# yellofi/SelectiveNet_for_semantic_segmentation_binary

Measured on AMD Instinct MI355X. Metric: train images/sec, SelectiveUNet_B 256x256 bs=128 (global), selective_loss s_lamb=2, higher is better.
Workload: dtype f32; 1 GPU; SelectiveUNet_B train step, global bs=128, 256x256, Adam lr=1e-3, s_lamb=2; model=SelectiveUNet_B, global_batch=128, per_gpu_batch=128, image=256, parallelism=dp1

## Files before the change

### selectivenet_for_semantic_segmentation_binary_amd/csrc/conv3x3.hip

```cpp
#include <cstdlib>

#include "gemm_common.h"

namespace selunet {

constexpr int TH = 16, TW = 16;
constexpr int HHT = TH + 2, HWT = TW + 2;
constexpr int HPIX = HHT * HWT;
constexpr int HTHREADS = 512;
constexpr int A_ROUNDS = (HPIX * 8 + HTHREADS - 1) / HTHREADS;
constexpr int AROWB = 160;
__device__ __forceinline__ int halo_off(int hp, int cc) { return hp * AROWB + ((cc ^ ((hp / HWT) & 1)) << 4); }

template <typename T, int BN, bool ONE_CHUNK>
__global__ void __launch_bounds__(HTHREADS, ONE_CHUNK ? 2 : 1)
conv3x3_halo_kernel(GatherArg g, const T* __restrict__ B, int N, int k_pad, EpiArg ep, int n_tiles, int tiles_x,
                    int tiles_y) {
  constexpr int E = 16 / sizeof(T);
  constexpr int CK = 128 / sizeof(T);
  constexpr int WAVES_N = BN / 64;
  constexpr int WAVES_M = 8 / WAVES_N;
  constexpr int WPIX = (TH * TW) / WAVES_M;
  constexpr int MT = WPIX / 32;
  constexpr int NT = 2;
// ... 1174 lines not shown
    __builtin_memcpy(&v, e, 16);
    return v;
  };
  uint4 rp[P_ROUNDS], rx[X_ROUNDS];
  auto load_tile = [&](int pt) __attribute__((always_inline)) {
    int img, y0, x0;
    tile_origin(pt, img, y0, x0);
#pragma unroll
    for (int r = 0; r < P_ROUNDS; ++r) {
      const int idx = r * 512 + tid;
      const int px = idx / (BI / 8), cc = idx % (BI / 8);
      const int y = min(y0 + px / WTW, H - 1), x = min(x0 + px % WTW, W - 1);
      rp[r] = *reinterpret_cast<const uint4*>(reinterpret_cast<const __bf16*>(pa.data) +
                                             (((int64_t)img * H + y) * W + x) * pa.C + i0 + cc * 8);
    }
#pragma unroll
    for (int r = 0; r < X_ROUNDS; ++r) {
      const int idx = r * 512 + tid;
      const int hp = min(idx >> 3, WHP - 1), cc = idx & 7;
      const int y = min(max(y0 - 1 + hp / WHW, 0), H - 1), x = min(max(x0 - 1 + hp % WHW, 0), W - 1);
      rx[r] = *reinterpret_cast<const uint4*>(reinterpret_cast<const __bf16*>(xa.data) +
                                             (((int64_t)img * H + y) * W + x) * xa.C + xc + cc * 8);
    }
  };
  auto store_tile = [&](int pt, int buf) __attribute__((always_inline)) {
    int img, y0, x0;
    tile_origin(pt, img, y0, x0);
#pragma unroll
    for (int r = 0; r < P_ROUNDS; ++r) {
      const int idx = r * 512 + tid;
      const int px = idx / (BI / 8), cc = idx % (BI / 8);
      uint4 v = make_uint4(0, 0, 0, 0);
      if (y0 + px / WTW < H && x0 + px % WTW < W)
        v = pa.scale ? apply(rp[r], Ks + cc * 8, Ks + BI + cc * 8, pa.relu) : rp[r];
      *reinterpret_cast<uint4*>(&Ps[buf][px][cc * 8]) = v;
    }
#pragma unroll
    for (int r = 0; r < X_ROUNDS; ++r) {
      const int idx = r * 512 + tid;
      if (idx < WHP * 8) {
        const int hp = idx >> 3, cc = idx & 7;
        const int y = y0 - 1 + hp / WHW, x = x0 - 1 + hp % WHW;
        uint4 v = make_uint4(0, 0, 0, 0);
        if ((unsigned)y < (unsigned)H && (unsigned)x < (unsigned)W)
          v = xa.scale ? apply(rx[r], Ks + 2 * BI + cc * 8, Ks + 2 * BI + 64 + cc * 8, xa.relu) : rx[r];
        *reinterpret_cast<uint4*>(&Xs[buf][hp][cc * 8]) = v;
      }
    }
  };

  f32x16 acc[NTAP];
#pragma unroll
  for (int t = 0; t < NTAP; ++t) acc[t] = f32x16{};

  load_tile((int)pt_begin);
  __syncthreads();
  store_tile((int)pt_begin, 0);
  __syncthreads();
  auto tile_loop = [&](auto ntc) __attribute__((always_inline)) {
    constexpr int NTP = decltype(ntc)::value;
    int buf = 0;
    for (int pt = (int)pt_begin; pt < (int)pt_end; ++pt) {
      const bool more = pt + 1 < (int)pt_end;
      load_tile(more ? pt + 1 : pt);
      __builtin_amdgcn_sched_barrier(0);
  #pragma unroll
      for (int ks = 0; ks < WTH; ++ks) {
        const int prow = ks * WTW + 8 * half + q4;
        const int pcol = wi * 32 + 16 * grp_hi + 4 * p4;
        s16x4 lo = __builtin_amdgcn_ds_read_tr16_b64_v4i16((__attribute__((address_space(3))) s16x4*)&Ps[buf][prow][pcol]);
        s16x4 hi = __builtin_amdgcn_ds_read_tr16_b64_v4i16((__attribute__((address_space(3))) s16x4*)&Ps[buf][prow + 4][pcol]);
        const bf16x8 af = __builtin_bit_cast(bf16x8, __builtin_shufflevector(lo, hi, 0, 1, 2, 3, 4, 5, 6, 7));
        const int xcol = wj * 32 + 16 * grp_hi + 4 * p4;
        constexpr int PF = 3;
        auto read_tap = [&](int t) __attribute__((always_inline)) {
          const int tap = min(tap0 + t, 8);
          const int dy = tap / 3, dx = tap - (tap / 3) * 3;
          const int xrow = (ks + dy) * WHW + 8 * half + dx + q4;
          s16x4 blo = __builtin_amdgcn_ds_read_tr16_b64_v4i16((__attribute__((address_space(3))) s16x4*)&Xs[buf][xrow][xcol]);
          s16x4 bhi = __builtin_amdgcn_ds_read_tr16_b64_v4i16((__attribute__((address_space(3))) s16x4*)&Xs[buf][xrow + 4][xcol]);
          return __builtin_bit_cast(bf16x8, __builtin_shufflevector(blo, bhi, 0, 1, 2, 3, 4, 5, 6, 7));
        };
        bf16x8 bfr[NTAP];
  #pragma unroll
        for (int t = 0; t < PF && t < NTAP; ++t) bfr[t] = read_tap(t);
        __builtin_amdgcn_sched_group_barrier(0x100, 2 + 2 * PF, 0);
  #pragma unroll
        for (int t = 0; t < NTAP; ++t) {
          if (t < NTP) acc[t] = __builtin_amdgcn_mfma_f32_32x32x16_bf16(af, bfr[t], acc[t], 0, 0, 0);
          __builtin_amdgcn_sched_group_barrier(0x008, 1, 0);
          if (t + PF < NTAP) {
            bfr[t + PF] = read_tap(t + PF);
            __builtin_amdgcn_sched_group_barrier(0x100, 2, 0);
          }
        }
      }
      if (more) store_tile(pt + 1, buf ^ 1);
      __syncthreads();
      buf ^= 1;
    }
  };
  if (TG == 1) tile_loop(std::integral_constant<int, 9>{});
  else if (tg == 0) tile_loop(std::integral_constant<int, 5>{});
  else tile_loop(std::integral_constant<int, 4>{});

  const int ctot = Q.Ctot;
#pragma unroll
  for (int t = 0; t < NTAP; ++t) {
    if (t < ntap) {
      const int tap = tap0 + t;
      const int j = tap * ctot + c0 + wj * 32 + l32;
#pragma unroll
      for (int r = 0; r < 16; ++r) {
        const int i = i0 + wi * 32 + (r & 3) + 8 * (r >> 2) + 4 * half;
        if (ws) ws[split * ws_stride + (int64_t)i * ldo + j] = acc[t][r];
        else atomicAdd(out + (int64_t)i * ldo + j, acc[t][r]);
      }
    }
  }
}

constexpr int XTH = 8, XTW = 8, XHW = XTW + 2, XHP = (XTH + 2) * XHW, XPIX = XTH * XTW;

template <int BI, int BNA = 0, bool TQ = false>
__global__ void __launch_bounds__(512, 1)
conv3x3_wgrad_x2_kernel(GatherArg P, GatherArg Q, int ldo, int co_tiles, int ci_chunks, int64_t tiles_per_split,
                        int tiles_x, int tiles_y, int64_t total_tiles, float* __restrict__ ws, int64_t ws_stride,
                        const float* __restrict__ amax_p, const float* __restrict__ amax_q0,
                        const float* __restrict__ amax_q1, WgradBnArg bn, unsigned* __restrict__ tq = nullptr) {
  constexpr int LDP = BI + 32;
  constexpr int LDX = 64 + 32;
  constexpr int TG = BI == 64 ? 2 : 1;
  constexpr int NTAP = TG == 1 ? 9 : 5;
  constexpr int P_ROUNDS = (XPIX * BI / 4) / 512;
  constexpr int X_ROUNDS = (XHP * 16 + 511) / 512;
  constexpr bool POOL = BNA == 2, HEADS = BNA == 3;
  constexpr int KX = BNA ? (HEADS ? 8 : 5) * BI : 2 * BI;
  constexpr int NWIN = XPIX * BI / 16;
  static_assert(P_ROUNDS * 512 == XPIX * BI / 4, "dY tile must split evenly over the threads");
  static_assert(!(POOL || HEADS) || (BI == 64 && NWIN <= 512), "pool / heads sources are BI = 64 forms");

  __shared__ __attribute__((aligned(16))) _Float16 Ps[2][2][XPIX][LDP];
  __shared__ __attribute__((aligned(16))) _Float16 Xs[2][2][XHP][LDX];
  __shared__ __attribute__((aligned(16))) float Ks[KX + 2 * 64];

  const int tid = threadIdx.x;
  const int lane = tid & 63, wave = tid >> 6;
  const int wj = wave & 1;
  const int wi = (wave >> 1) % (BI / 32);
  const int tg = (wave >> 1) / (BI / 32);
  const int tap0 = tg * 5;
  const int ntap = TG == 1 ? 9 : (tg == 0 ? 5 : 4);
  const int half = lane >> 5, l32 = lane & 31;
  const int grp_hi = (lane >> 4) & 1, q4 = (lane & 15) >> 2, p4 = lane & 3;

  const unsigned lb = xcd_remap(blockIdx.x, gridDim.x);
  const int cot = lb % co_tiles;
  const int rest = lb / co_tiles;
  const int cik = rest % ci_chunks;
  const int64_t split = rest / ci_chunks;
  const int i0 = cot * BI;
  const int c0 = cik * 64;
  const int ngroups = co_tiles * ci_chunks, grp = (int)(lb % (unsigned)ngroups);
  __shared__ int tq_slot[2];
  int pt_first, pt_second, pt_stop;
  if constexpr (TQ) {
    if (tid == 0) {
      const unsigned t = atomicAdd(tq + grp, 2u);
      tq_slot[0] = (int)min(t, (unsigned)total_tiles);
      tq_slot[1] = (int)min(t + 1u, (unsigned)total_tiles);
    }
    __syncthreads();
    pt_first = tq_slot[0];
    pt_second = tq_slot[1];
    pt_stop = (int)total_tiles;
  } else {
    pt_first = (int)(split * tiles_per_split);
    pt_second = pt_first + 1;
    pt_stop = (int)min(total_tiles, (int64_t)pt_first + tiles_per_split);
  }

  int xs_src = 0, xc = c0;
  if (Q.nsrc > 1 && xc >= Q.src[0].C) {
    xc -= Q.src[0].C;
    xs_src = 1;
  }
  const SrcArg xa = pick_src(Q, xs_src);
  const SrcArg& pa = P.src[0];
  const int H = P.h, W = P.w;
  float uns_p, uns_x;
  const float sp = x2_scale(amax_p[0], &uns_p);
  const float sx = x2_scale((xs_src ? amax_q1 : amax_q0)[0], &uns_x);

  if constexpr (BNA) {
    for (int k = tid; k < KX; k += 512) {
      const int c = i0 + (k % BI), C = P.Ctot;
      float v;
      switch (k / BI) {
        case 0: v = bn.scale[c]; break;
        case 1: v = bn.shift[c]; break;
        case 2: v = bn.coef[c]; break;
        case 3: v = bn.coef[2 * C + c] * bn.invstd[c]; break;
        case 4: v = bn.coef[C + c] - bn.coef[2 * C + c] * bn.invstd[c] * bn.mean[c]; break;
        default: {
          const int hd = k / BI - 5;
          v = hd < bn.nh ? bn.hw[hd * 64 + c] : 0.0f;
        }
      }
      Ks[k] = v;
    }
    if (tid < 128) {
      const int c = xc + (tid % 64);
      Ks[KX + tid] = xa.scale ? (tid < 64 ? xa.scale[c] : xa.shift[c]) : 0.0f;
    }
  } else if (tid < 2 * BI + 128) {
    float v;
    if (tid < 2 * BI) {
      const int c = i0 + (tid % BI);
      v = pa.scale ? (tid < BI ? pa.scale[c] : pa.shift[c]) : 0.0f;
    } else {
      const int c = xc + ((tid - 2 * BI) % 64);
      v = xa.scale ? (tid < 2 * BI + 64 ? xa.scale[c] : xa.shift[c]) : 0.0f;
    }
    Ks[tid] = v;
  }
  float dam = 0.0f;
  const bool dy_out = BNA && bn.dy != nullptr;

  constexpr int PPR = 512 / (BI / 4);
  const int hrem = H - (tiles_y - 1) * XTH, wrem = W - (tiles_x - 1) * XTW;
  const int pcc = tid % (BI / 4);
  unsigned tb = 0, p_off, g_off = 0, w_off = 0, x_off[X_ROUNDS];
  if constexpr (POOL) {
    const int wn = tid / (BI / 4), wyy = 2 * (wn / (XTW / 2)), wxx = 2 * (wn % (XTW / 2));
    p_off = (unsigned)((wyy * W + wxx) * pa.C + pcc * 4) * 4u;
    w_off = (unsigned)(((wyy / 2) * (W / 2) + wxx / 2) * pa.C + pcc * 4) * 4u;
    if (wyy >= hrem) tb |= 1u << 16;
    if (wxx >= wrem) tb |= 1u << 20;
#pragma unroll
    for (int k = 0; k < 4; ++k)
      if (((wyy + (k >> 1)) * XTW + wxx + (k & 1)) % ci_chunks == cik) tb |= 1u << (24 + k);
  } else {
    const int px = tid / (BI / 4), py = px / XTW, pxx = px % XTW;
    p_off = (unsigned)((py * W + pxx) * pa.C + pcc * 4) * 4u;
    if constexpr (HEADS) g_off = (unsigned)(py * W + pxx) * 4u;
    if (pxx >= wrem) tb |= 1u << 20;
#pragma unroll
    for (int r = 0; r < P_ROUNDS; ++r) {
      if (py + r * (PPR / XTW) >= hrem) tb |= 1u << (16 + r);
      if (BNA && (r * PPR + px) % ci_chunks == cik) tb |= 1u << (24 + r);
    }
  }
#pragma unroll
  for (int r = 0; r < X_ROUNDS; ++r) {
    const int hp = min((r * 512 + tid) >> 4, XHP - 1), hy = hp / XHW, hx = hp % XHW;
    x_off[r] = (unsigned)((hy * W + hx) * xa.C + (tid & 15) * 4) * 4u;
    tb |= (unsigned)((hy == 0) | (hy > hrem) << 1 | (hx == 0) << 2 | (hx > wrem) << 3) << (4 * r);
  }
  const unsigned p_rstride = (unsigned)((PPR / XTW) * W * pa.C) * 4u;
  const unsigned g_rstride = (unsigned)((PPR / XTW) * W) * 4u;
  const unsigned x_safe = (unsigned)((W + 1) * xa.C) * 4u;
  struct Geo {
    int64_t pix;
    int64_t hpix;
    unsigned em;
  };
  auto tile_geo = [&](int pt_) __attribute__((always_inline)) {
    const unsigned pt = (unsigned)__builtin_amdgcn_readfirstlane(pt_);
    const unsigned r2 = pt / (unsigned)tiles_x, tx = pt - r2 * (unsigned)tiles_x;
    const unsigned r3 = r2 / (unsigned)tiles_y, ty = r2 - r3 * (unsigned)tiles_y;
    Geo g;
    g.pix = ((int64_t)r3 * H + ty * XTH) * W + tx * XTW;
    g.hpix = POOL ? ((int64_t)r3 * (H / 2) + ty * (XTH / 2)) * (W / 2) + tx * (XTW / 2) : 0;
    g.em = (ty == 0 ? 0x1111u : 0u) | (ty == (unsigned)tiles_y - 1u ? 0x0f2222u : 0u) |
           (tx == 0 ? 0x4444u : 0u) | (tx == (unsigned)tiles_x - 1u ? 0x108888u : 0u);
    return g;
  };
  auto p_in = [&](const Geo& g, int r) __attribute__((always_inline)) {
    return (tb & g.em & ((POOL ? 1u << 16 : 1u << (16 + r)) | 1u << 20)) == 0;
  };
  auto x_in = [&](const Geo& g, int r) __attribute__((always_inline)) { return (tb & g.em & (0xfu << (4 * r))) == 0; };
  auto at = [&](const void* base, int64_t elems, unsigned off) __attribute__((always_inline)) {
    return reinterpret_cast<const char*>(reinterpret_cast<const float*>(base) + elems) + (size_t)off;
  };
  auto put = [&](float4 v, const float* sc, const float* sh, int relu, float s, _Float16* hp, _Float16* lp)
      __attribute__((always_inline)) {
    float f[4] = {v.x, v.y, v.z, v.w};
    f16x4 h, l;
#pragma unroll
    for (int j = 0; j < 4; ++j) {
      float t = f[j];
      if (sc) {
        t = t * sc[j] + sh[j];
        if (relu) t = fmaxf(t, 0.0f);
      }
      _Float16 a, b;
      x2_split(t * s, a, b);
      h[j] = a;
      l[j] = b;
    }
    *reinterpret_cast<f16x4*>(hp) = h;
    *reinterpret_cast<f16x4*>(lp) = l;
  };
  float4 rp[P_ROUNDS], rx[X_ROUNDS];
  float4 ry[BNA ? P_ROUNDS : 1];
  float rg[HEADS ? P_ROUNDS : 1][3];
  float4 wy[POOL ? 4 : 1], wk[POOL ? 4 : 1], wg;
  auto load_p = [&](const Geo& g, int r0, int r1) __attribute__((always_inline)) {
    const int64_t e0 = g.pix * pa.C + i0;
    if constexpr (POOL) {
      if (r0 == 0 && tid < NWIN) {
        const bool in = p_in(g, 0);
        const unsigned o = in ? p_off : 0u;
        const int64_t rs = (int64_t)W * pa.C;
        const int64_t ek[4] = {e0, e0 + pa.C, e0 + rs, e0 + rs + pa.C};
#pragma unroll
        for (int k = 0; k < 4; ++k) {
          wy[k] = *reinterpret_cast<const float4*>(at(bn.y, ek[k], o));
          wk[k] = bn.skip ? *reinterpret_cast<const float4*>(at(bn.skip, ek[k], o)) : make_float4(0, 0, 0, 0);
        }
        wg = *reinterpret_cast<const float4*>(at(bn.pooled, g.hpix * pa.C + i0, in ? w_off : 0u));
      }
      return;
    }
#pragma unroll
    for (int r = 0; r < P_ROUNDS; ++r) {
      if (r < r0 || r >= r1) continue;
      const bool in = p_in(g, r);
      const unsigned o = in ? p_off + r * p_rstride : 0u;
      if constexpr (HEADS) {
        const unsigned go = in ? g_off + r * g_rstride : 0u;
        rg[r][0] = *reinterpret_cast<const float*>(at(bn.g0, g.pix, go));
        rg[r][1] = bn.nh > 1 ? *reinterpret_cast<const float*>(at(bn.g1, g.pix, go)) : 0.0f;
        rg[r][2] = bn.nh > 1 ? *reinterpret_cast<const float*>(at(bn.g2, g.pix, go)) : 0.0f;
      } else {
        rp[r] = *reinterpret_cast<const float4*>(at(pa.data, e0, o));
      }
      if constexpr (BNA) ry[r] = *reinterpret_cast<const float4*>(at(bn.y, e0, o));
    }
  };
  auto load_x = [&](const Geo& g) __attribute__((always_inline)) {
    const int64_t e0 = (g.pix - W - 1) * xa.C + xc;
#pragma unroll
    for (int r = 0; r < X_ROUNDS; ++r)
      rx[r] = *reinterpret_cast<const float4*>(at(xa.data, e0, x_in(g, r) ? x_off[r] : x_safe));
  };
  auto store_p = [&](const Geo& tl, int buf, int r0, int r1) __attribute__((always_inline)) {
    const int64_t e0 = tl.pix * pa.C + i0;
    if constexpr (POOL) {
      if (r0 == 0 && tid < NWIN) {
        const int wi = tid / (BI / 4), cg = tid % (BI / 4);
        const int wyy = 2 * (wi / (XTW / 2)), wxx = 2 * (wi % (XTW / 2));
        const bool in = p_in(tl, 0);
        const f32x4 csc = *reinterpret_cast<const f32x4*>(Ks + cg * 4);
        const f32x4 csh = *reinterpret_cast<const f32x4*>(Ks + BI + cg * 4);
        const f32x4 ck0 = *reinterpret_cast<const f32x4*>(Ks + 2 * BI + cg * 4);
        const f32x4 ca = *reinterpret_cast<const f32x4*>(Ks + 3 * BI + cg * 4);
        const f32x4 cb = *reinterpret_cast<const f32x4*>(Ks + 4 * BI + cg * 4);
        const float yv[4][4] = {{wy[0].x, wy[0].y, wy[0].z, wy[0].w}, {wy[1].x, wy[1].y, wy[1].z, wy[1].w},
                                {wy[2].x, wy[2].y, wy[2].z, wy[2].w}, {wy[3].x, wy[3].y, wy[3].z, wy[3].w}};
        const float gv[4] = {wg.x, wg.y, wg.z, wg.w};
        int arg[4] = {0, 0, 0, 0};
#pragma unroll
        for (int e = 0; e < 4; ++e) {
          float best = fmaxf(yv[0][e] * csc[e] + csh[e], 0.0f);
#pragma unroll
          for (int k = 1; k < 4; ++k) {
            const float v = fmaxf(yv[k][e] * csc[e] + csh[e], 0.0f);
            if (v > best) {
              best = v;
              arg[e] = k;
            }
          }
        }
#pragma unroll
        for (int k = 0; k < 4; ++k) {
          float d[4] = {wk[k].x, wk[k].y, wk[k].z, wk[k].w};
          float o[4];
#pragma unroll
          for (int e = 0; e < 4; ++e) {
            if (arg[e] == k) d[e] += gv[e];
            o[e] = (yv[k][e] * csc[e] + csh[e] > 0.0f ? ck0[e] * d[e] : 0.0f) - cb[e] - ca[e] * yv[k][e];
          }
          const int py = wyy + (k >> 1), pxx = wxx + (k & 1), px = py * XTW + pxx;
          const float4 dv = in ? make_float4(o[0], o[1], o[2], o[3]) : make_float4(0, 0, 0, 0);
          if (dy_out && in && (tb & (1u << (24 + k)))) {
            const int64_t ek = e0 + ((k >> 1) * (int64_t)W + (k & 1)) * pa.C;
            *reinterpret_cast<float4*>(const_cast<char*>(at(bn.dy, ek, p_off))) = dv;
            dam = fmaxf(dam, fmaxf(fmaxf(fabsf(dv.x), fabsf(dv.y)), fmaxf(fabsf(dv.z), fabsf(dv.w))));
          }
          put(dv, nullptr, nullptr, 0, sp, &Ps[buf][0][px][cg * 4], &Ps[buf][1][px][cg * 4]);
        }
      }
      return;
    }
#pragma unroll
    for (int r = 0; r < P_ROUNDS; ++r) {
      if (r < r0 || r >= r1) continue;
      const int idx = r * 512 + tid;
      const int px = idx / (BI / 4), cc = idx % (BI / 4);
      const bool in = p_in(tl, r);
      if constexpr (BNA) {
        float g[4] = {rp[r].x, rp[r].y, rp[r].z, rp[r].w};
        const float yv[4] = {ry[r].x, ry[r].y, ry[r].z, ry[r].w};
        if constexpr (HEADS) {
          const f32x4 w0 = *reinterpret_cast<const f32x4*>(Ks + 5 * BI + cc * 4);
          const f32x4 w1 = *reinterpret_cast<const f32x4*>(Ks + 6 * BI + cc * 4);
          const f32x4 w2 = *reinterpret_cast<const f32x4*>(Ks + 7 * BI + cc * 4);
#pragma unroll
          for (int e = 0; e < 4; ++e) g[e] = w0[e] * rg[r][0] + w1[e] * rg[r][1] + w2[e] * rg[r][2];
        }
        const f32x4 csc = *reinterpret_cast<const f32x4*>(Ks + cc * 4);
        const f32x4 csh = *reinterpret_cast<const f32x4*>(Ks + BI + cc * 4);
        const f32x4 ck0 = *reinterpret_cast<const f32x4*>(Ks + 2 * BI + cc * 4);
        const f32x4 ca = *reinterpret_cast<const f32x4*>(Ks + 3 * BI + cc * 4);
        const f32x4 cb = *reinterpret_cast<const f32x4*>(Ks + 4 * BI + cc * 4);
        float o[4];
#pragma unroll
        for (int e = 0; e < 4; ++e)
          o[e] = (yv[e] * csc[e] + csh[e] > 0.0f ? ck0[e] * g[e] : 0.0f) - cb[e] - ca[e] * yv[e];
        const float4 d = in ? make_float4(o[0], o[1], o[2], o[3]) : make_float4(0, 0, 0, 0);
        if (dy_out && in && (tb & (1u << (24 + r)))) {
          *reinterpret_cast<float4*>(const_cast<char*>(at(bn.dy, e0 + r * (int64_t)(p_rstride / 4), p_off))) = d;
          dam = fmaxf(dam, fmaxf(fmaxf(fabsf(d.x), fabsf(d.y)), fmaxf(fabsf(d.z), fabsf(d.w))));
        }
        put(d, nullptr, nullptr, 0, sp, &Ps[buf][0][px][cc * 4], &Ps[buf][1][px][cc * 4]);
      } else {
        put(in ? rp[r] : make_float4(0, 0, 0, 0), pa.scale && in ? Ks + cc * 4 : nullptr, Ks + BI + cc * 4, pa.relu,
            sp, &Ps[buf][0][px][cc * 4], &Ps[buf][1][px][cc * 4]);
      }
    }
  };
  auto store_x = [&](const Geo& g, int buf) __attribute__((always_inline)) {
#pragma unroll
    for (int r = 0; r < X_ROUNDS; ++r) {
      const int idx = r * 512 + tid;
      if (idx < XHP * 16) {
        const int hp = idx >> 4, cc = idx & 15;
        const bool in = x_in(g, r);
        put(in ? rx[r] : make_float4(0, 0, 0, 0), xa.scale && in ? Ks + KX + cc * 4 : nullptr,
            Ks + KX + 64 + cc * 4, xa.relu, sx, &Xs[buf][0][hp][cc * 4], &Xs[buf][1][hp][cc * 4]);
      }
    }
  };

  f32x16 acc[NTAP];
#pragma unroll
  for (int t = 0; t < NTAP; ++t) acc[t] = f32x16{};

  if (pt_first < pt_stop) {
    const Geo g0 = tile_geo(pt_first);
    load_p(g0, 0, P_ROUNDS);
    load_x(g0);
    __syncthreads();
    store_p(g0, 0, 0, P_ROUNDS);
    store_x(g0, 0);
    __syncthreads();
  }
  typedef __attribute__((address_space(3))) s16x4 lds_s16x4;
  auto tr8 = [&](const _Float16* p0, const _Float16* p1) __attribute__((always_inline)) {
    s16x4 lo = __builtin_amdgcn_ds_read_tr16_b64_v4i16((lds_s16x4*)p0);
    s16x4 hi = __builtin_amdgcn_ds_read_tr16_b64_v4i16((lds_s16x4*)p1);
    return __builtin_bit_cast(f16x8, __builtin_shufflevector(lo, hi, 0, 1, 2, 3, 4, 5, 6, 7));
  };
  auto tile_loop = [&](auto ntc) __attribute__((always_inline)) {
    constexpr int NTP = decltype(ntc)::value;
    int buf = 0;
    int pt_tq = pt_second;
    for (int pt = pt_first; pt < pt_stop;) {
      const int ptn = TQ ? pt_tq : pt + 1;
      const bool more = ptn < pt_stop;
      unsigned claimed = 0;
      constexpr bool QSPLIT = BNA && BI == 128;
      constexpr int PH = QSPLIT ? P_ROUNDS / 2 : P_ROUNDS;
      const Geo gn = tile_geo(more ? ptn : pt);
      load_p(gn, 0, PH);
      __builtin_amdgcn_sched_barrier(0);
#pragma unroll
      for (int ks = 0; ks < XPIX / 16; ++ks) {
        if (QSPLIT && ks == 1) {
          if (more) store_p(gn, buf ^ 1, 0, PH);
          load_p(gn, PH, P_ROUNDS);
          __builtin_amdgcn_sched_barrier(0);
        }
        if (BI == 64 && ks == 1) {
          load_x(gn);
          __builtin_amdgcn_sched_barrier(0);
        }
        if (ks == (QSPLIT || BI == 64 ? 3 : 2)) {
          if (more) store_p(gn, buf ^ 1, QSPLIT ? PH : 0, P_ROUNDS);
          if (BI != 64) load_x(gn);
          __builtin_amdgcn_sched_barrier(0);
        }
        if constexpr (TQ) {
          if (ks == 0 && tid == 0) claimed = atomicAdd(tq + grp, 1u);
        }
        const int prow = ks * 16 + 8 * half + q4;
        const int pcol = wi * 32 + 16 * grp_hi + 4 * p4;
        const f16x8 ah = tr8(&Ps[buf][0][prow][pcol], &Ps[buf][0][prow + 4][pcol]);
        const f16x8 al = tr8(&Ps[buf][1][prow][pcol], &Ps[buf][1][prow + 4][pcol]);
        const int xcol = wj * 32 + 16 * grp_hi + 4 * p4;
        constexpr int PF = BI == 128 ? 1 : 2;
        struct Frag {
          f16x8 h, l;
        };
        auto read_tap = [&](int t) __attribute__((always_inline)) {
          constexpr int TAP0 = TG == 2 && NTP == 4 ? 5 : 0;
          const int tap = min(TAP0 + t, 8);
          const int dy = tap / 3, dx = tap - (tap / 3) * 3;
          const int xrow = (2 * ks + half + dy) * XHW + dx + q4;
          Frag f;
          f.h = tr8(&Xs[buf][0][xrow][xcol], &Xs[buf][0][xrow + 4][xcol]);
          f.l = tr8(&Xs[buf][1][xrow][xcol], &Xs[buf][1][xrow + 4][xcol]);
          return f;
        };
        Frag bfr[NTAP];
#pragma unroll
        for (int t = 0; t < PF && t < NTAP; ++t) bfr[t] = read_tap(t);
        __builtin_amdgcn_sched_group_barrier(0x100, 4 + 4 * PF, 0);
#pragma unroll
        for (int t = 0; t < NTAP; ++t) {
          if (t < NTP) {
            acc[t] = __builtin_amdgcn_mfma_f32_32x32x16_f16(ah, bfr[t].l, acc[t], 0, 0, 0);
            acc[t] = __builtin_amdgcn_mfma_f32_32x32x16_f16(al, bfr[t].h, acc[t], 0, 0, 0);
            acc[t] = __builtin_amdgcn_mfma_f32_32x32x16_f16(ah, bfr[t].h, acc[t], 0, 0, 0);
          }
          __builtin_amdgcn_sched_group_barrier(0x008, 3, 0);
          if (t + PF < NTAP) {
            bfr[t + PF] = read_tap(t + PF);
            __builtin_amdgcn_sched_group_barrier(0x100, 4, 0);
          }
        }
      }
      if constexpr (TQ) {
        if (tid == 0) tq_slot[buf] = (int)min(claimed, (unsigned)pt_stop);
      }
      if (more) store_x(gn, buf ^ 1);
      __syncthreads();
      if constexpr (TQ) pt_tq = tq_slot[buf];
      pt = ptn;
      buf ^= 1;
    }
  };
  if (TG == 1) tile_loop(std::integral_constant<int, 9>{});
  else if (tg == 0) tile_loop(std::integral_constant<int, 5>{});
  else tile_loop(std::integral_constant<int, 4>{});

  if constexpr (BNA) {
    if (bn.dy_amax) block_amax(bn.dy_amax, dam, Ks);
  }
  if constexpr (TQ) {
    const unsigned splits = gridDim.x / (unsigned)ngroups;
    if (tid == 0 && atomicAdd(tq + ngroups + grp, 1u) == splits - 1u) {
      atomicExch(tq + grp, 0u);
      atomicExch(tq + ngroups + grp, 0u);
    }
  }
  const float ofac = uns_p * uns_x;
  const int ctot = Q.Ctot;
#pragma unroll
  for (int t = 0; t < NTAP; ++t) {
    if (t < ntap) {
      const int tap = tap0 + t;
      const int j = tap * ctot + c0 + wj * 32 + l32;
#pragma unroll
      for (int r = 0; r < 16; ++r) {
        const int i = i0 + wi * 32 + (r & 3) + 8 * (r >> 2) + 4 * half;
        ws[split * ws_stride + (int64_t)i * ldo + j] = acc[t][r] * ofac;
      }
    }
  }
}

constexpr int FTH = 8, FTW = 8;

template <int BI, int WCO>
__global__ void __launch_bounds__(512, 1)
conv3x3_wgrad_halo_f32_kernel(GatherArg P, GatherArg Q, float* __restrict__ out, int ldo, int co_tiles,
                              int ci_chunks, int64_t tiles_per_split, int tiles_x, int tiles_y, int64_t total_tiles,
                              float* __restrict__ ws, int64_t ws_stride) {
  constexpr int CJ = 64;
  constexpr int WTH = FTH, WTW = FTW, WHW = FTW + 2, WPIXT = FTH * FTW, WHP = (FTH + 2) * (FTW + 2);
  constexpr int NT = 512;
  constexpr int MA = WCO / 32;
  constexpr int COH = BI / WCO;
  constexpr int TGN = 8 / (COH * 2);
  static_assert(TGN == 2 || TGN == 4, "8 waves = co groups x 2 ci halves x tap groups");
  constexpr int NTAP = TGN == 2 ? 5 : 3;
  constexpr int P_ROUNDS = (WPIXT * BI / 4) / NT;
  constexpr int X_ROUNDS = (WHP * (CJ / 4) + NT - 1) / NT;
  constexpr int KS = WPIXT / 2;
  constexpr int UNR = BI == 128 ? 2 : 4;
  static_assert(P_ROUNDS * NT == WPIXT * BI / 4, "dY tile must split evenly over the threads");

  __shared__ __attribute__((aligned(16))) float Ps[2][WPIXT][BI];
  __shared__ __attribute__((aligned(16))) float Xs[2][WHP][CJ];
  __shared__ float Ks[2 * BI + 2 * CJ];

  const int tid = threadIdx.x;
  const int lane = tid & 63, wave = tid >> 6;
  const int wj = wave & 1;
  const int wc = (wave >> 1) % COH;
  const int tg = (wave >> 1) / COH;
  const int tap0 = TGN == 2 ? tg * 5 : (tg == 0 ? 0 : 1 + 2 * tg);
  const int ntap = TGN == 2 ? (tg == 0 ? 5 : 4) : (tg == 0 ? 3 : 2);
  const int half = lane >> 5, l32 = lane & 31;

  const unsigned lb = xcd_remap(blockIdx.x, gridDim.x);
  const int cot = lb % co_tiles;
  const int rest = lb / co_tiles;
  const int cik = rest % ci_chunks;
  const int64_t split = rest / ci_chunks;
  const int i0 = cot * BI;
  const int c0 = cik * CJ;
  const int64_t pt_begin = split * tiles_per_split;
  const int64_t pt_end = min(total_tiles, pt_begin + tiles_per_split);
  if (pt_begin >= pt_end) return;

  int xs_src = 0, xc = c0;
  if (Q.nsrc > 1 && xc >= Q.src[0].C) {
    xc -= Q.src[0].C;
    xs_src = 1;
  }
  const SrcArg xa = pick_src(Q, xs_src);
  const SrcArg& pa = P.src[0];
  const int H = P.h, W = P.w;

  if (tid < 2 * BI + 2 * CJ) {
    float v;
    if (tid < 2 * BI) {
      const int c = i0 + (tid % BI);
      v = pa.scale ? (tid < BI ? pa.scale[c] : pa.shift[c]) : 0.0f;
    } else {
      const int c = xc + ((tid - 2 * BI) % CJ);
      v = xa.scale ? (tid < 2 * BI + CJ ? xa.scale[c] : xa.shift[c]) : 0.0f;
    }
    Ks[tid] = v;
  }

  auto tile_origin = [&](int pt, int& img, int& y0, int& x0) __attribute__((always_inline)) {
    const unsigned r2 = (unsigned)pt / (unsigned)tiles_x;
    x0 = ((unsigned)pt - r2 * (unsigned)tiles_x) * WTW;
    const unsigned r3 = r2 / (unsigned)tiles_y;
    y0 = (r2 - r3 * (unsigned)tiles_y) * WTH;
    img = (int)r3;
  };
  auto apply = [&](f32x4 v, const float* sc, const float* sh, int relu) __attribute__((always_inline)) {
#pragma unroll
    for (int j = 0; j < 4; ++j) {
      const float f = v[j] * sc[j] + sh[j];
      v[j] = relu ? fmaxf(f, 0.0f) : f;
    }
    return v;
  };
  f32x4 rp[P_ROUNDS], rx[X_ROUNDS];
  auto load_p = [&](int pt) __attribute__((always_inline)) {
    int img, y0, x0;
    tile_origin(pt, img, y0, x0);
#pragma unroll
    for (int r = 0; r < P_ROUNDS; ++r) {
      const int idx = r * NT + tid;
      const int px = idx / (BI / 4), cc = idx % (BI / 4);
      const int y = min(y0 + px / WTW, H - 1), x = min(x0 + px % WTW, W - 1);
      rp[r] = *reinterpret_cast<const f32x4*>(reinterpret_cast<const float*>(pa.data) +
                                              (((int64_t)img * H + y) * W + x) * pa.C + i0 + cc * 4);
    }
  };
  auto load_x = [&](int pt) __attribute__((always_inline)) {
    int img, y0, x0;
    tile_origin(pt, img, y0, x0);
#pragma unroll
    for (int r = 0; r < X_ROUNDS; ++r) {
      const int idx = r * NT + tid;
      const int hp = min(idx >> 4, WHP - 1), cc = idx & 15;
      const int y = min(max(y0 - 1 + hp / WHW, 0), H - 1), x = min(max(x0 - 1 + hp % WHW, 0), W - 1);
      rx[r] = *reinterpret_cast<const f32x4*>(reinterpret_cast<const float*>(xa.data) +
                                              (((int64_t)img * H + y) * W + x) * xa.C + xc + cc * 4);
    }
  };
  auto store_p = [&](int pt, int buf) __attribute__((always_inline)) {
    int img, y0, x0;
    tile_origin(pt, img, y0, x0);
#pragma unroll
    for (int r = 0; r < P_ROUNDS; ++r) {
      const int idx = r * NT + tid;
      const int px = idx / (BI / 4), cc = idx % (BI / 4);
      f32x4 v = {0.0f, 0.0f, 0.0f, 0.0f};
      if (y0 + px / WTW < H && x0 + px % WTW < W)
        v = pa.scale ? apply(rp[r], Ks + cc * 4, Ks + BI + cc * 4, pa.relu) : rp[r];
      *reinterpret_cast<f32x4*>(&Ps[buf][px][cc * 4]) = v;
    }
  };
  auto store_x = [&](int pt, int buf) __attribute__((always_inline)) {
    int img, y0, x0;
    tile_origin(pt, img, y0, x0);
#pragma unroll
    for (int r = 0; r < X_ROUNDS; ++r) {
      const int idx = r * NT + tid;
      if (idx < WHP * (CJ / 4)) {
        const int hp = idx >> 4, cc = idx & 15;
        const int y = y0 - 1 + hp / WHW, x = x0 - 1 + hp % WHW;
        f32x4 v = {0.0f, 0.0f, 0.0f, 0.0f};
        if ((unsigned)y < (unsigned)H && (unsigned)x < (unsigned)W)
          v = xa.scale ? apply(rx[r], Ks + 2 * BI + cc * 4, Ks + 2 * BI + CJ + cc * 4, xa.relu) : rx[r];
        *reinterpret_cast<f32x4*>(&Xs[buf][hp][cc * 4]) = v;
      }
    }
  };

  f32x16 acc[MA][NTAP];
#pragma unroll
  for (int a = 0; a < MA; ++a)
#pragma unroll
    for (int t = 0; t < NTAP; ++t) acc[a][t] = f32x16{};

  int toff[NTAP];
#pragma unroll
  for (int t = 0; t < NTAP; ++t) {
    const int tap = min(tap0 + t, 8);
    toff[t] = ((tap / 3) * WHW + tap % 3) * CJ;
  }
  struct Frag {
    float a[MA], b[NTAP];
  };
  auto frag = [&](int buf, int ks) __attribute__((always_inline)) {
    Frag f;
    const int p = 2 * ks + half;
    const float* pr = &Ps[buf][p][wc * WCO + l32];
#pragma unroll
    for (int a = 0; a < MA; ++a) f.a[a] = pr[a * 32];
    const float* xr = &Xs[buf][(p / WTW) * WHW + p % WTW][wj * 32 + l32];
#pragma unroll
    for (int t = 0; t < NTAP; ++t) f.b[t] = xr[toff[t]];
    return f;
  };

  load_p((int)pt_begin);
  load_x((int)pt_begin);
  __syncthreads();
  store_p((int)pt_begin, 0);
  store_x((int)pt_begin, 0);
  __syncthreads();
  int buf = 0;
  for (int pt = (int)pt_begin; pt < (int)pt_end; ++pt) {
    const bool more = pt + 1 < (int)pt_end;
    if (more) { load_p(pt + 1); load_x(pt + 1); }
    Frag cur = frag(buf, 0);
#pragma unroll UNR
    for (int ks = 0; ks < KS; ++ks) {
      const Frag nxt = frag(buf, ks + 1 < KS ? ks + 1 : 0);
#pragma unroll
      for (int t = 0; t < NTAP; ++t)
        if (t < ntap) {
#pragma unroll
          for (int a = 0; a < MA; ++a)
            acc[a][t] = __builtin_amdgcn_mfma_f32_32x32x2f32(cur.a[a], cur.b[t], acc[a][t], 0, 0, 0);
        }

      cur = nxt;
    }
    if (more) { store_p(pt + 1, buf ^ 1); store_x(pt + 1, buf ^ 1); }
    __syncthreads();
    buf ^= 1;
  }

  int ln = lane;
  asm volatile("" : "+v"(ln));
  const int ctot = Q.Ctot;
#pragma unroll
  for (int t = 0; t < NTAP; ++t) {
    if (t < ntap) {
      const int tap = tap0 + t;
      const int j = tap * ctot + c0 + wj * 32 + (ln & 31);
#pragma unroll
      for (int a = 0; a < MA; ++a)
#pragma unroll
        for (int r = 0; r < 16; ++r) {
          const int i = i0 + wc * WCO + a * 32 + (r & 3) + 8 * (r >> 2) + 4 * (ln >> 5);
          if (ws) ws[split * ws_stride + (int64_t)i * ldo + j] = acc[a][t][r];
          else atomicAdd(out + (int64_t)i * ldo + j, acc[a][t][r]);
        }
    }
  }
}

template <int TWW, int NW>
__global__ void __launch_bounds__(NW * 64, 1)
conv3x3_wgrad_wino_f32_kernel(GatherArg P, GatherArg Q, int co_tiles, int ci_chunks, int64_t tiles_per_split,
                              int tiles_x, int tiles_y, int64_t total_tiles, float* __restrict__ ws, int64_t ws_stride,
                              int ldw) {
  constexpr int BI = 64, CJ = 64;
  constexpr int WTH = FTH, WTW = TWW, WHW = TWW + 2, WPIXT = FTH * TWW, WHP = (FTH + 2) * (TWW + 2);
  constexpr int NT = NW * 64;
  constexpr int P_VEC = WPIXT * BI / 4;
  constexpr int P_ROUNDS = (P_VEC + NT - 1) / NT;
  constexpr int X_ROUNDS = (WHP * (CJ / 4) + NT - 1) / NT;
  constexpr int NACC = NW == 8 ? 6 : 4;
  constexpr int KS = WPIXT / 4;
  constexpr int PPR = TWW / 2;
  static_assert(NW == 8 || NW == 12, "8 or 12 waves");

  __shared__ __attribute__((aligned(16))) float Ps[2][WPIXT][BI];
  __shared__ __attribute__((aligned(16))) float Xs[2][WHP][CJ];
  __shared__ float Ks[2 * BI + 2 * CJ];

  const int tid = threadIdx.x;
  const int lane = tid & 63, wave = tid >> 6;
  const int wj = wave & 1;
  const int wc = (wave >> 1) & 1;
  const int tg = wave >> 2;
  const int half = lane >> 5, l32 = lane & 31;

  const unsigned lb = xcd_remap(blockIdx.x, gridDim.x);
  const int cot = lb % co_tiles;
  const int rest = lb / co_tiles;
  const int cik = rest % ci_chunks;
  const int64_t split = rest / ci_chunks;
  const int i0 = cot * BI;
  const int c0 = cik * CJ;
  const int64_t pt_begin = split * tiles_per_split;
  const int64_t pt_end = min(total_tiles, pt_begin + tiles_per_split);

  int xs_src = 0, xc = c0;
  if (Q.nsrc > 1 && xc >= Q.src[0].C) {
    xc -= Q.src[0].C;
    xs_src = 1;
  }
  const SrcArg xa = pick_src(Q, xs_src);
  const SrcArg& pa = P.src[0];
  const int H = P.h, W = P.w;

  if (tid < 2 * BI + 2 * CJ) {
    float v;
    if (tid < 2 * BI) {
      const int c = i0 + (tid % BI);
      v = pa.scale ? (tid < BI ? pa.scale[c] : pa.shift[c]) : 0.0f;
    } else {
      const int c = xc + ((tid - 2 * BI) % CJ);
      v = xa.scale ? (tid < 2 * BI + CJ ? xa.scale[c] : xa.shift[c]) : 0.0f;
    }
    Ks[tid] = v;
  }

  auto tile_origin = [&](int pt, int& img, int& y0, int& x0) __attribute__((always_inline)) {
    const unsigned r2 = (unsigned)pt / (unsigned)tiles_x;
    x0 = ((unsigned)pt - r2 * (unsigned)tiles_x) * WTW;
    const unsigned r3 = r2 / (unsigned)tiles_y;
    y0 = (r2 - r3 * (unsigned)tiles_y) * WTH;
    img = (int)r3;
// ... 467 lines not shown
```

Before: 1432 images/s.

## Add two-stage register prefetch pipeline to BI=64 conv3x3 weight-gradient kernel

For the BI==64, non-queue weight-gradient path, global loads for the P and X operands are now issued two tiles ahead into alternating register stage structs. Their LDS stores for the next tile are spread round by round across the k-steps using a compile-time schedule table. The main loop is unrolled by two so the buffer indices are compile-time constants. The goal is to hide global-load latency behind the MFMA work, at the cost of doubled staging registers, which may lower occupancy or cause spills.

```diff
diff --git a/selectivenet_for_semantic_segmentation_binary_amd/csrc/conv3x3.hip b/selectivenet_for_semantic_segmentation_binary_amd/csrc/conv3x3.hip
--- a/selectivenet_for_semantic_segmentation_binary_amd/csrc/conv3x3.hip
+++ b/selectivenet_for_semantic_segmentation_binary_amd/csrc/conv3x3.hip
@@ -1500,11 +1500,16 @@
     *reinterpret_cast<f16x4*>(hp) = h;
     *reinterpret_cast<f16x4*>(lp) = l;
   };
-  float4 rp[P_ROUNDS], rx[X_ROUNDS];
-  float4 ry[BNA ? P_ROUNDS : 1];
-  float rg[HEADS ? P_ROUNDS : 1][3];
-  float4 wy[POOL ? 4 : 1], wk[POOL ? 4 : 1], wg;
-  auto load_p = [&](const Geo& g, int r0, int r1) __attribute__((always_inline)) {
+  struct PStage {
+    float4 rp[P_ROUNDS];
+    float4 ry[BNA ? P_ROUNDS : 1];
+    float rg[HEADS ? P_ROUNDS : 1][3];
+    float4 wy[POOL ? 4 : 1], wk[POOL ? 4 : 1], wg;
+  };
+  struct XStage {
+    float4 rx[X_ROUNDS];
+  };
+  auto load_p = [&](PStage& S, const Geo& g, int r0, int r1) __attribute__((always_inline)) {
     const int64_t e0 = g.pix * pa.C + i0;
     if constexpr (POOL) {
       if (r0 == 0 && tid < NWIN) {
@@ -1514,10 +1519,10 @@
         const int64_t ek[4] = {e0, e0 + pa.C, e0 + rs, e0 + rs + pa.C};
 #pragma unroll
         for (int k = 0; k < 4; ++k) {
-          wy[k] = *reinterpret_cast<const float4*>(at(bn.y, ek[k], o));
-          wk[k] = bn.skip ? *reinterpret_cast<const float4*>(at(bn.skip, ek[k], o)) : make_float4(0, 0, 0, 0);
-        }
-        wg = *reinterpret_cast<const float4*>(at(bn.pooled, g.hpix * pa.C + i0, in ? w_off : 0u));
+          S.wy[k] = *reinterpret_cast<const float4*>(at(bn.y, ek[k], o));
+          S.wk[k] = bn.skip ? *reinterpret_cast<const float4*>(at(bn.skip, ek[k], o)) : make_float4(0, 0, 0, 0);
+        }
+        S.wg = *reinterpret_cast<const float4*>(at(bn.pooled, g.hpix * pa.C + i0, in ? w_off : 0u));
       }
       return;
     }
@@ -1528,22 +1533,22 @@
       const unsigned o = in ? p_off + r * p_rstride : 0u;
       if constexpr (HEADS) {
         const unsigned go = in ? g_off + r * g_rstride : 0u;
-        rg[r][0] = *reinterpret_cast<const float*>(at(bn.g0, g.pix, go));
-        rg[r][1] = bn.nh > 1 ? *reinterpret_cast<const float*>(at(bn.g1, g.pix, go)) : 0.0f;
-        rg[r][2] = bn.nh > 1 ? *reinterpret_cast<const float*>(at(bn.g2, g.pix, go)) : 0.0f;
+        S.rg[r][0] = *reinterpret_cast<const float*>(at(bn.g0, g.pix, go));
+        S.rg[r][1] = bn.nh > 1 ? *reinterpret_cast<const float*>(at(bn.g1, g.pix, go)) : 0.0f;
+        S.rg[r][2] = bn.nh > 1 ? *reinterpret_cast<const float*>(at(bn.g2, g.pix, go)) : 0.0f;
       } else {
-        rp[r] = *reinterpret_cast<const float4*>(at(pa.data, e0, o));
-      }
-      if constexpr (BNA) ry[r] = *reinterpret_cast<const float4*>(at(bn.y, e0, o));
-    }
-  };
-  auto load_x = [&](const Geo& g) __attribute__((always_inline)) {
+        S.rp[r] = *reinterpret_cast<const float4*>(at(pa.data, e0, o));
+      }
+      if constexpr (BNA) S.ry[r] = *reinterpret_cast<const float4*>(at(bn.y, e0, o));
+    }
+  };
+  auto load_x = [&](XStage& S, const Geo& g) __attribute__((always_inline)) {
     const int64_t e0 = (g.pix - W - 1) * xa.C + xc;
 #pragma unroll
     for (int r = 0; r < X_ROUNDS; ++r)
-      rx[r] = *reinterpret_cast<const float4*>(at(xa.data, e0, x_in(g, r) ? x_off[r] : x_safe));
-  };
-  auto store_p = [&](const Geo& tl, int buf, int r0, int r1) __attribute__((always_inline)) {
+      S.rx[r] = *reinterpret_cast<const float4*>(at(xa.data, e0, x_in(g, r) ? x_off[r] : x_safe));
+  };
+  auto store_p = [&](const PStage& S, const Geo& tl, int buf, int r0, int r1) __attribute__((always_inline)) {
     const int64_t e0 = tl.pix * pa.C + i0;
     if constexpr (POOL) {
       if (r0 == 0 && tid < NWIN) {
@@ -1555,9 +1560,10 @@
         const f32x4 ck0 = *reinterpret_cast<const f32x4*>(Ks + 2 * BI + cg * 4);
         const f32x4 ca = *reinterpret_cast<const f32x4*>(Ks + 3 * BI + cg * 4);
         const f32x4 cb = *reinterpret_cast<const f32x4*>(Ks + 4 * BI + cg * 4);
+        const float4* wy = S.wy;
         const float yv[4][4] = {{wy[0].x, wy[0].y, wy[0].z, wy[0].w}, {wy[1].x, wy[1].y, wy[1].z, wy[1].w},
                                 {wy[2].x, wy[2].y, wy[2].z, wy[2].w}, {wy[3].x, wy[3].y, wy[3].z, wy[3].w}};
-        const float gv[4] = {wg.x, wg.y, wg.z, wg.w};
+        const float gv[4] = {S.wg.x, S.wg.y, S.wg.z, S.wg.w};
         int arg[4] = {0, 0, 0, 0};
 #pragma unroll
         for (int e = 0; e < 4; ++e) {
@@ -1573,7 +1579,7 @@
         }
 #pragma unroll
         for (int k = 0; k < 4; ++k) {
-          float d[4] = {wk[k].x, wk[k].y, wk[k].z, wk[k].w};
+          float d[4] = {S.wk[k].x, S.wk[k].y, S.wk[k].z, S.wk[k].w};
           float o[4];
 #pragma unroll
           for (int e = 0; e < 4; ++e) {
@@ -1599,14 +1605,14 @@
       const int px = idx / (BI / 4), cc = idx % (BI / 4);
       const bool in = p_in(tl, r);
       if constexpr (BNA) {
-        float g[4] = {rp[r].x, rp[r].y, rp[r].z, rp[r].w};
-        const float yv[4] = {ry[r].x, ry[r].y, ry[r].z, ry[r].w};
+        float g[4] = {S.rp[r].x, S.rp[r].y, S.rp[r].z, S.rp[r].w};
+        const float yv[4] = {S.ry[r].x, S.ry[r].y, S.ry[r].z, S.ry[r].w};
         if constexpr (HEADS) {
           const f32x4 w0 = *reinterpret_cast<const f32x4*>(Ks + 5 * BI + cc * 4);
           const f32x4 w1 = *reinterpret_cast<const f32x4*>(Ks + 6 * BI + cc * 4);
           const f32x4 w2 = *reinterpret_cast<const f32x4*>(Ks + 7 * BI + cc * 4);
 #pragma unroll
-          for (int e = 0; e < 4; ++e) g[e] = w0[e] * rg[r][0] + w1[e] * rg[r][1] + w2[e] * rg[r][2];
+          for (int e = 0; e < 4; ++e) g[e] = w0[e] * S.rg[r][0] + w1[e] * S.rg[r][1] + w2[e] * S.rg[r][2];
         }
         const f32x4 csc = *reinterpret_cast<const f32x4*>(Ks + cc * 4);
         const f32x4 csh = *reinterpret_cast<const f32x4*>(Ks + BI + cc * 4);
@@ -1624,19 +1630,19 @@
         }
         put(d, nullptr, nullptr, 0, sp, &Ps[buf][0][px][cc * 4], &Ps[buf][1][px][cc * 4]);
       } else {
-        put(in ? rp[r] : make_float4(0, 0, 0, 0), pa.scale && in ? Ks + cc * 4 : nullptr, Ks + BI + cc * 4, pa.relu,
+        put(in ? S.rp[r] : make_float4(0, 0, 0, 0), pa.scale && in ? Ks + cc * 4 : nullptr, Ks + BI + cc * 4, pa.relu,
             sp, &Ps[buf][0][px][cc * 4], &Ps[buf][1][px][cc * 4]);
       }
     }
   };
-  auto store_x = [&](const Geo& g, int buf) __attribute__((always_inline)) {
+  auto store_x = [&](const XStage& S, const Geo& g, int buf, int r0 = 0, int r1 = X_ROUNDS) __attribute__((always_inline)) {
 #pragma unroll
     for (int r = 0; r < X_ROUNDS; ++r) {
       const int idx = r * 512 + tid;
-      if (idx < XHP * 16) {
+      if (r >= r0 && r < r1 && idx < XHP * 16) {
         const int hp = idx >> 4, cc = idx & 15;
         const bool in = x_in(g, r);
-        put(in ? rx[r] : make_float4(0, 0, 0, 0), xa.scale && in ? Ks + KX + cc * 4 : nullptr,
+        put(in ? S.rx[r] : make_float4(0, 0, 0, 0), xa.scale && in ? Ks + KX + cc * 4 : nullptr,
             Ks + KX + 64 + cc * 4, xa.relu, sx, &Xs[buf][0][hp][cc * 4], &Xs[buf][1][hp][cc * 4]);
       }
     }
@@ -1646,13 +1652,34 @@
 #pragma unroll
   for (int t = 0; t < NTAP; ++t) acc[t] = f32x16{};
 
+#ifndef SELUNET_WGRAD64_PIPE
+#define SELUNET_WGRAD64_PIPE 1
+#endif
+#ifndef SELUNET_WGRAD64_STAGE
+#define SELUNET_WGRAD64_STAGE 1
+#endif
+  constexpr bool PIPE_X = SELUNET_WGRAD64_PIPE && BI == 64 && !TQ;
+  constexpr bool PIPE_P = PIPE_X && !POOL;
+#ifdef SELUNET_ABL_WGRAD_HOT
+  constexpr bool ABL_HOT = true;
+#else
+  constexpr bool ABL_HOT = false;
+#endif
+  PStage pA, pB;
+  XStage xA, xB;
   if (pt_first < pt_stop) {
     const Geo g0 = tile_geo(pt_first);
-    load_p(g0, 0, P_ROUNDS);
-    load_x(g0);
+    load_p(pA, g0, 0, P_ROUNDS);
+    load_x(xA, g0);
+    if constexpr (PIPE_X) {
+      const Geo gb = tile_geo(!ABL_HOT && pt_second < pt_stop ? pt_second : pt_first);
+      if constexpr (PIPE_P) load_p(pB, gb, 0, P_ROUNDS);
+      load_x(xB, gb);
+      __builtin_amdgcn_sched_barrier(0);
+    }
     __syncthreads();
-    store_p(g0, 0, 0, P_ROUNDS);
-    store_x(g0, 0);
+    store_p(pA, g0, 0, 0, P_ROUNDS);
+    store_x(xA, g0, 0);
     __syncthreads();
   }
   typedef __attribute__((address_space(3))) s16x4 lds_s16x4;
@@ -1661,8 +1688,46 @@
     s16x4 hi = __builtin_amdgcn_ds_read_tr16_b64_v4i16((lds_s16x4*)p1);
     return __builtin_bit_cast(f16x8, __builtin_shufflevector(lo, hi, 0, 1, 2, 3, 4, 5, 6, 7));
   };
+  auto mma_step = [&](auto ntc, int ks, int buf) __attribute__((always_inline)) {
+    constexpr int NTP = decltype(ntc)::value;
+    const int prow = ks * 16 + 8 * half + q4;
+    const int pcol = wi * 32 + 16 * grp_hi + 4 * p4;
+    const f16x8 ah = tr8(&Ps[buf][0][prow][pcol], &Ps[buf][0][prow + 4][pcol]);
+    const f16x8 al = tr8(&Ps[buf][1][prow][pcol], &Ps[buf][1][prow + 4][pcol]);
+    const int xcol = wj * 32 + 16 * grp_hi + 4 * p4;
+    constexpr int PF = BI == 128 ? 1 : 2;
+    struct Frag {
+      f16x8 h, l;
+    };
+    auto read_tap = [&](int t) __attribute__((always_inline)) {
+      constexpr int TAP0 = TG == 2 && NTP == 4 ? 5 : 0;
+      const int tap = min(TAP0 + t, 8);
+      const int dy = tap / 3, dx = tap - (tap / 3) * 3;
+      const int xrow = (2 * ks + half + dy) * XHW + dx + q4;
+      Frag f;
+      f.h = tr8(&Xs[buf][0][xrow][xcol], &Xs[buf][0][xrow + 4][xcol]);
+      f.l = tr8(&Xs[buf][1][xrow][xcol], &Xs[buf][1][xrow + 4][xcol]);
+      return f;
+    };
+    Frag bfr[NTAP];
+#pragma unroll
+    for (int t = 0; t < PF && t < NTAP; ++t) bfr[t] = read_tap(t);
+    __builtin_amdgcn_sched_group_barrier(0x100, 4 + 4 * PF, 0);
+#pragma unroll
+    for (int t = 0; t < NTAP; ++t) {
+      if (t < NTP) {
+        acc[t] = __builtin_amdgcn_mfma_f32_32x32x16_f16(ah, bfr[t].l, acc[t], 0, 0, 0);
+        acc[t] = __builtin_amdgcn_mfma_f32_32x32x16_f16(al, bfr[t].h, acc[t], 0, 0, 0);
+        acc[t] = __builtin_amdgcn_mfma_f32_32x32x16_f16(ah, bfr[t].h, acc[t], 0, 0, 0);
+      }
+      __builtin_amdgcn_sched_group_barrier(0x008, 3, 0);
+      if (t + PF < NTAP) {
+        bfr[t + PF] = read_tap(t + PF);
+        __builtin_amdgcn_sched_group_barrier(0x100, 4, 0);
+      }
+    }
+  };
   auto tile_loop = [&](auto ntc) __attribute__((always_inline)) {
-    constexpr int NTP = decltype(ntc)::value;
     int buf = 0;
     int pt_tq = pt_second;
     for (int pt = pt_first; pt < pt_stop;) {
@@ -1672,77 +1737,107 @@
       constexpr bool QSPLIT = BNA && BI == 128;
       constexpr int PH = QSPLIT ? P_ROUNDS / 2 : P_ROUNDS;
       const Geo gn = tile_geo(more ? ptn : pt);
-      load_p(gn, 0, PH);
+      const Geo gl = ABL_HOT ? tile_geo(pt_first) : gn;
+      load_p(pA, gl, 0, PH);
       __builtin_amdgcn_sched_barrier(0);
 #pragma unroll
       for (int ks = 0; ks < XPIX / 16; ++ks) {
         if (QSPLIT && ks == 1) {
-          if (more) store_p(gn, buf ^ 1, 0, PH);
-          load_p(gn, PH, P_ROUNDS);
+          if (more) store_p(pA, gn, buf ^ 1, 0, PH);
+          load_p(pA, gl, PH, P_ROUNDS);
           __builtin_amdgcn_sched_barrier(0);
         }
         if (BI == 64 && ks == 1) {
-          load_x(gn);
+          load_x(xA, gl);
           __builtin_amdgcn_sched_barrier(0);
         }
         if (ks == (QSPLIT || BI == 64 ? 3 : 2)) {
-          if (more) store_p(gn, buf ^ 1, QSPLIT ? PH : 0, P_ROUNDS);
-          if (BI != 64) load_x(gn);
+          if (more) store_p(pA, gn, buf ^ 1, QSPLIT ? PH : 0, P_ROUNDS);
+          if (BI != 64) load_x(xA, gl);
           __builtin_amdgcn_sched_barrier(0);
         }
         if constexpr (TQ) {
           if (ks == 0 && tid == 0) claimed = atomicAdd(tq + grp, 1u);
         }
-        const int prow = ks * 16 + 8 * half + q4;
-        const int pcol = wi * 32 + 16 * grp_hi + 4 * p4;
-        const f16x8 ah = tr8(&Ps[buf][0][prow][pcol], &Ps[buf][0][prow + 4][pcol]);
-        const f16x8 al = tr8(&Ps[buf][1][prow][pcol], &Ps[buf][1][prow + 4][pcol]);
-        const int xcol = wj * 32 + 16 * grp_hi + 4 * p4;
-        constexpr int PF = BI == 128 ? 1 : 2;
-        struct Frag {
-          f16x8 h, l;
-        };
-        auto read_tap = [&](int t) __attribute__((always_inline)) {
-          constexpr int TAP0 = TG == 2 && NTP == 4 ? 5 : 0;
-          const int tap = min(TAP0 + t, 8);
-          const int dy = tap / 3, dx = tap - (tap / 3) * 3;
-          const int xrow = (2 * ks + half + dy) * XHW + dx + q4;
-          Frag f;
-          f.h = tr8(&Xs[buf][0][xrow][xcol], &Xs[buf][0][xrow + 4][xcol]);
-          f.l = tr8(&Xs[buf][1][xrow][xcol], &Xs[buf][1][xrow + 4][xcol]);
-          return f;
-        };
-        Frag bfr[NTAP];
-#pragma unroll
-        for (int t = 0; t < PF && t < NTAP; ++t) bfr[t] = read_tap(t);
-        __builtin_amdgcn_sched_group_barrier(0x100, 4 + 4 * PF, 0);
-#pragma unroll
-        for (int t = 0; t < NTAP; ++t) {
-          if (t < NTP) {
-            acc[t] = __builtin_amdgcn_mfma_f32_32x32x16_f16(ah, bfr[t].l, acc[t], 0, 0, 0);
-            acc[t] = __builtin_amdgcn_mfma_f32_32x32x16_f16(al, bfr[t].h, acc[t], 0, 0, 0);
-            acc[t] = __builtin_amdgcn_mfma_f32_32x32x16_f16(ah, bfr[t].h, acc[t], 0, 0, 0);
-          }
-          __builtin_amdgcn_sched_group_barrier(0x008, 3, 0);
-          if (t + PF < NTAP) {
-            bfr[t + PF] = read_tap(t + PF);
-            __builtin_amdgcn_sched_group_barrier(0x100, 4, 0);
-          }
-        }
+        mma_step(ntc, ks, buf);
       }
       if constexpr (TQ) {
         if (tid == 0) tq_slot[buf] = (int)min(claimed, (unsigned)pt_stop);
       }
-      if (more) store_x(gn, buf ^ 1);
+      if (more) store_x(xA, gn, buf ^ 1);
       __syncthreads();
       if constexpr (TQ) pt_tq = tq_slot[buf];
       pt = ptn;
       buf ^= 1;
     }
   };
-  if (TG == 1) tile_loop(std::integral_constant<int, 9>{});
-  else if (tg == 0) tile_loop(std::integral_constant<int, 5>{});
-  else tile_loop(std::integral_constant<int, 4>{});
+  auto tile_loop2 = [&](auto ntc) __attribute__((always_inline)) {
+    Geo g1 = tile_geo(pt_second < pt_stop ? pt_second : pt_first);
+    constexpr int SCH[2][2][6] = {{{3, 3, 4, 4, 4, 4}, {3, 3, 4, 4, 4, 4}},
+                                  {{0, 1, 2, 2, 3, 3}, {1, 1, 3, 3, 3, 3}}};
+    constexpr int TGI = decltype(ntc)::value == 5 ? 0 : 1;
+    auto p_at = [](int r, int ks) constexpr { return (PIPE_P ? SCH[SELUNET_WGRAD64_STAGE][TGI][r] : 3) == ks; };
+    auto x_at = [](int r, int ks) constexpr { return SCH[SELUNET_WGRAD64_STAGE][TGI][2 + r] == ks; };
+    auto tile = [&](int pt, auto bufc, auto morec, PStage& pn, XStage& xn, PStage& pf, XStage& xf)
+        __attribute__((always_inline)) {
+      constexpr int buf = decltype(bufc)::value;
+      const bool more = decltype(morec)::value || pt + 1 < pt_stop;
+      const Geo g2 = tile_geo(pt + 2 < pt_stop ? pt + 2 : pt);
+      const Geo gl = ABL_HOT ? tile_geo(pt_first) : g2;
+      if constexpr (PIPE_P) load_p(pf, gl, 0, P_ROUNDS);
+      else load_p(pn, ABL_HOT ? gl : g1, 0, P_ROUNDS);
+      __builtin_amdgcn_sched_barrier(0);
+      auto stage = [&](int ks) __attribute__((always_inline)) {
+        bool any = false;
+#pragma unroll
+        for (int r = 0; r < X_ROUNDS; ++r) any |= x_at(r, ks) || (r < P_ROUNDS && p_at(r, ks));
+        if (!any) return;
+        if (more) {
+          if constexpr (POOL) {
+            if (p_at(0, ks)) store_p(pn, g1, buf ^ 1, 0, P_ROUNDS);
+          } else {
+#pragma unroll
+            for (int r = 0; r < P_ROUNDS; ++r)
+              if (p_at(r, ks)) store_p(pn, g1, buf ^ 1, r, r + 1);
+          }
+#pragma unroll
+          for (int r = 0; r < X_ROUNDS; ++r)
+            if (x_at(r, ks)) store_x(xn, g1, buf ^ 1, r, r + 1);
+        }
+        __builtin_amdgcn_sched_barrier(0);
+      };
+#pragma unroll
+      for (int ks = 0; ks < XPIX / 16; ++ks) {
+        if (ks == 1) {
+          load_x(xf, gl);
+          __builtin_amdgcn_sched_barrier(0);
+        }
+        stage(ks);
+        mma_step(ntc, ks, buf);
+      }
+      stage(XPIX / 16);
+      __syncthreads();
+      g1 = g2;
+    };
+    int pt = pt_first;
+    for (; pt + 1 < pt_stop; pt += 2) {
+      tile(pt, std::integral_constant<int, 0>{}, std::true_type{}, PIPE_P ? pB : pA, xB, pA, xA);
+      tile(pt + 1, std::integral_constant<int, 1>{}, std::false_type{}, pA, xA, PIPE_P ? pB : pA, xB);
+    }
+    if (pt < pt_stop) {
+#pragma unroll
+      for (int ks = 0; ks < XPIX / 16; ++ks) mma_step(ntc, ks, 0);
+      __syncthreads();
+    }
+  };
+  if constexpr (PIPE_X) {
+    if (tg == 0) tile_loop2(std::integral_constant<int, 5>{});
+    else tile_loop2(std::integral_constant<int, 4>{});
+  } else {
+    if (TG == 1) tile_loop(std::integral_constant<int, 9>{});
+    else if (tg == 0) tile_loop(std::integral_constant<int, 5>{});
+    else tile_loop(std::integral_constant<int, 4>{});
+  }
 
   if constexpr (BNA) {
     if (bn.dy_amax) block_amax(bn.dy_amax, dam, Ks);
```

Result: no change. 1436 images/s (median of 6 runs) (+0.3%).
